# lmchion/PowerGridworld

Measured on AMD Instinct MI355X. Metric: agent-env-steps/sec at batch 65536, 5-agent scenario, 1/2/4/8 MI355X, higher is better.
Workload: dtype f64; 1 GPU; C4: 5-agent coordinated buildings (building+PV+storage) + IEEE-13 power flow + voltage-violation reward; pf_convergence=opendss, batch_per_gpu=65536, global_batch=65536, episode_steps=286, parallelism=env-sharded x1 (no collective on the step path)

## Files before the change

powergridworld_amd/csrc/pgw_pf.hip:

```cpp
#include <algorithm>
#include <cstdlib>
#include <cmath>
#include <type_traits>
#include <atomic>
#include <vector>

#include "pgw_common.h"

static std::atomic<bool> g_pf_trace_on{false};

namespace pgw {

template <int B, int E, class F>
__device__ __forceinline__ void static_for(F&& f) {
  if constexpr (B < E) {
    f(std::integral_constant<int, B>{});
    static_for<B + 1, E>(f);
  }
}

template <int M> struct PFBlock {
  static constexpr int kTri = M * (M + 1) / 2;
  static constexpr int kU0re = 3 * kTri, kU0im = kU0re + M, kU0sum = kU0im + M;
  static constexpr int kLo2 = kU0sum + M, kMn2 = kLo2 + M, kMx2 = kMn2 + M;
// ... 1740 lines not shown
    }
#pragma unroll
    for (int q = 0; q < kRq; ++q) {
      const int x = x0 + lane + 64 * q;
      if (x < z.n_rows * S) sh.rows[(x / S) * kWaveRowStride + (x - (x / S) * S)] = v[q];
    }
  }
  __builtin_amdgcn_fence(__ATOMIC_RELEASE, "wavefront");
  __builtin_amdgcn_wave_barrier();
  __builtin_amdgcn_fence(__ATOMIC_ACQUIRE, "wavefront");
}

__device__ __forceinline__ void od_wave_rows(const ODWaveShared& sh, int M, int r0, int r1, double pjr,
                                             double pji, double cjr, double cji, double& err, double& amin) {
  int lane = threadIdx.x & 63;
  asm volatile("" : "+v"(lane));
  const bool newer = lane >= 32;
  const int r = min(r0 + (lane & 31), max(r1 - 1, 0));
  const bool on = r0 + (lane & 31) < r1;
  const double* R = sh.rows + r * kWaveRowStride;
  double vr = R[0], vi = R[1];
#pragma unroll
  for (int k = 0; k < PGW_PF_MAX_M; ++k) {
    if (k >= M) break;
    const double gr = R[2 + k], gi = R[2 + M + k];
    const double pr = wave_bcast(pjr, k), pi = wave_bcast(pji, k);
    const double cr = wave_bcast(cjr, k), ci = wave_bcast(cji, k);
    const double jx = newer ? cr : pr, jy = newer ? ci : pi;
    vr = fma(gr, jx, vr);
    vi = fma(gr, jy, vi);
    vr = fma(-gi, jy, vr);
    vi = fma(gi, jx, vi);
  }
  const double mg = od_mag(fma(vi, vi, vr * vr));
  const double mn = wave_xor(mg, 32);
  const bool prev_lane = on && !newer;
  err = od_max(err, prev_lane ? fabs(mn - mg) : 0.0);
  amin = fmin(amin, prev_lane ? mg : __builtin_huge_val());
}

__device__ int od_wave_solve(const ODWaveArgs& z_, const ODWaveShared& sh_, double pc, double qc, double& v0r,
                             double& v0i) {
  int lane = threadIdx.x & 63;
  asm volatile("" : "+v"(lane));
  const ODWaveArgs& z = z_;
  const ODWaveShared& sh = sh_;
  const int M = z.m, T = M * (M + 1) / 2;
  const int i = min(lane, M - 1);
  const double sr0 = sh.el[0][i], si0 = sh.el[1][i], fr = sh.el[2][i], fi = sh.el[3][i];
  const double y0r = sh.el[4][i], y0i = sh.el[5][i], esc = sh.el[6][i];
  const bool node = lane < M && ((z.node_mask >> i) & 1);
  const double s_r = fma(fr, pc, sr0), s_i = fma(fi, qc, si0);
  const double* st = sh.st;
  const double u0re = sh.el[7][i], u0sum = sh.el[8][i];
  double ur = fma(qc, st[2 * (2 * M + i)], fma(pc, st[2 * (M + i)], st[2 * i]));
  double ui = fma(qc, st[2 * (2 * M + i) + 1], fma(pc, st[2 * (M + i) + 1], st[2 * i + 1]));
  const int c1 = 3 * M + i;
  double pjr = fma(qc, st[2 * (2 * M + c1)], fma(pc, st[2 * (M + c1)], st[2 * c1]));
  double pji = fma(qc, st[2 * (2 * M + c1) + 1], fma(pc, st[2 * (M + c1) + 1], st[2 * c1 + 1]));
  const double tol_lo = z.tol * (1.0 + 0x1p-30);
  const bool bounded = z.n_rep < z.n_rows;
  int it = 1, my_it = 1;
  bool conv_ok = false, done = z.max_iter <= 1;
  while (!done) {
    ++it;
    const double m2 = fma(ui, ui, ur * ur);
    double mc = fmin(fmax(m2, z.mn2), z.mx2);
    mc = (m2 <= z.lo2) ? 1.0 : mc;
    const double g = fast_rcp(mc);
    const double cr = fma(s_r, g, -y0r), ci = fma(s_i, g, -y0i);
    const double cjr = fma(cr, ur, -(ci * ui)), cji = fma(cr, ui, ci * ur);
    const double cjs = cjr + cji;
    double A = u0re, Bs = 0.0, C = u0sum;
    int ie = i;
    asm volatile("" : "+v"(ie));
    const double* wk = &sh.w[0][0][0] + ie;
#pragma unroll
    for (int k = 0; k < PGW_PF_MAX_M; ++k) {
      if (k < M) {
        A = fma(wk[k * PGW_PF_MAX_M], wave_bcast(cjr, k), A);
        Bs = fma(wk[(PGW_PF_MAX_M + k) * PGW_PF_MAX_M], wave_bcast(cji, k), Bs);
        C = fma(wk[(2 * PGW_PF_MAX_M + k) * PGW_PF_MAX_M], wave_bcast(cjs, k), C);
      }
    }
    const double nr = A - Bs, ni = (C - A) - Bs;
    bool hit = false;
    double err = 0.0, amin = __builtin_huge_val();
    {
      const double e2 = esc * esc;
      const double a2 = fma(ni, ni, nr * nr) * e2, b2 = fma(ui, ui, ur * ur) * e2;
      hit = node && fabs(a2 - b2) > tol_lo * fma(0.5, a2 + b2, 1.0);
    }
    const bool need = it >= z.min_iter && __ballot(hit) == 0ull;
    if (need) {
      const double mo = od_mag(fma(ui, ui, ur * ur)) * esc;
      const double mn = od_mag(fma(ni, ni, nr * nr)) * esc;
      err = node ? fabs(mn - mo) : 0.0;
      amin = node ? mo : __builtin_huge_val();
    }
    ur = nr;
    ui = ni;
    int d = 0;
    if (need) {
      double dsum = 0.0, jsum = 0.0;
#pragma unroll
      for (int k = 0; k < PGW_PF_MAX_M; ++k) {
        if (k >= M) break;
        const double cx = wave_bcast(cjr, k), cy = wave_bcast(cji, k);
        const double px = wave_bcast(pjr, k), py = wave_bcast(pji, k);
        dsum += fabs(cx - px) + fabs(cy - py);
        jsum += fabs(px) + fabs(py);
      }
      dsum = wave_uni(fma(0x1p-40, jsum + dsum, dsum));
      jsum = wave_uni(fma(0x1p-40, jsum, jsum));
      for (int r0 = 0; r0 < z.n_rep; r0 += 32)
        od_wave_rows(sh, M, r0, min(r0 + 32, z.n_rep), pjr, pji, cjr, cji, err, amin);
      double lo = wave_uni(wave_max(err)), am = wave_uni(wave_min(amin));
      d = __builtin_amdgcn_readfirstlane(od_decide(z, !bounded, it, lo, am, dsum, jsum));
      if (d < 0) {
        for (int r0 = z.n_rep; r0 < z.n_rows; r0 += 32)
          od_wave_rows(sh, M, r0, min(r0 + 32, z.n_rows), pjr, pji, cjr, cji, err, amin);
        lo = wave_uni(wave_max(err));
        am = wave_uni(wave_min(amin));
        d = __builtin_amdgcn_readfirstlane(od_decide(z, true, it, lo, am, dsum, jsum));
      }
    }
    pjr = cjr;
    pji = cji;
    my_it = it;
    conv_ok = d > 0;
    done = d > 0 || it >= z.max_iter;
  }
  const double* B = z.block + 3 * T + 6 * M;
  double vr = B[2 * M], vi = B[2 * M + 1];
#pragma unroll 4
  for (int k = 0; k < M; ++k) {
    const double gr = B[k], gi = B[M + k];
    const double jr = wave_bcast(pjr, k), ji = wave_bcast(pji, k);
    vr = fma(gr, jr, vr);
    vi = fma(gr, ji, vi);
    vr = fma(-gi, ji, vr);
    vi = fma(gi, jr, vi);
  }
  v0r = vr;
  v0i = vi;
  return conv_ok ? my_it : -my_it;
}

struct StepOdArgs {
  pgw_coord_params p;
  ODWaveArgs z;
};
template <bool WT, bool INL>
__global__ void __launch_bounds__(64 * PGW_MAX_AGENTS) __attribute__((amdgpu_waves_per_eu(7))) k_coord_step_od(StepOdArgs A_, pgw_coord_step_info s,
                                                                       int64_t n, pgw_coord_buffers b, double pv_ob,
                                                                       StdDerived dv, CoordPFArgs c, ODVLook o) {
  auto put = [](auto* q, auto v) {
    if constexpr (WT) st_wt(q, v);
    else *q = v;
  };
  const StepOdArgs& A = PGW_KERNARG0(StepOdArgs);
  const pgw_coord_params& p = A.p;
  const ODWaveArgs& z = A.z;
  const int a = threadIdx.x >> 6, lane = threadIdx.x & 63;
  const int64_t e = (int64_t)blockIdx.x * 64 + lane;
  const bool valid = e < n;
  __shared__ double s_pow[PGW_MAX_AGENTS][64];
  __shared__ double s_share[64];
  __shared__ int s_served[64];
  if (blockIdx.x == 0 && threadIdx.x == 0) b.od_count[(b.od_parity & 1) ^ 1] = 0;
  const ODVLook ol = {o.resp_v, o.resp_x0, o.resp_inv_h, o.resp_nseg, 0};
  double rw = 0.0;
  StdAgentInEarly in[1];
  double* xp = b.x + (int64_t)a * 5 * n + e;
  double* socp = b.soc + (int64_t)a * n + e;
  if (valid) {
    const double* ap = b.action.ptr + a * b.act_stride_agent + e * b.action.s_env;
#pragma unroll
    for (int j = 0; j < 8; ++j) in[0].av[j] = ld_act(ap + j * b.action.s_dim);
    in[0].soc = *socp;
#pragma unroll
    for (int z = 0; z < 5; ++z) in[0].xs[z] = xp[z * n];
    std_agent_compute<1, 1>(p, dv, s, pv_ob, in, [&](int, const double (&v)[1]) {
      s_pow[a][lane] = v[0];
      put(b.agent_power + (int64_t)a * n + e, v[0]);
    });
  }
  __syncthreads();
  double pc = 0.0;
  ODVRec rec;
  bool cell = false;
  if (valid) {
    double* op = b.obs.ptr + a * b.obs_stride_agent + e * b.obs.s_env;
    std_agent_compute<1, 2>(p, dv, s, pv_ob, in, [&](int slot, const double (&v)[1]) {
      if (slot < kSlotSoc) {
        put(xp + slot * n, v[0]);
        if (slot == kSlotX + 4 && a == 0) {
#pragma unroll
          for (int ag = 0; ag < PGW_MAX_AGENTS; ++ag) {
            const int cs = ag < c.n_agents ? c.agent_ctrl[ag] : -1;
            const double pa = ag < c.n_agents ? s_pow[ag][lane] * 1.0 : 0.0;
            pc = (cs == 0) ? pc + pa : pc;
          }
          int r = 0;
          cell = !o.timing_only && od_resp_v_cell(ol, pc, 0.0, r);
          if (cell) rec = od_resp_v_load(ol, r);
        }
      } else if (slot == kSlotSoc) put(socp, v[0]);
      else if (slot < kSlotPower) {
        if constexpr (WT) st_wt(op + (slot - kSlotObs) * b.obs.s_dim, v[0]);
        else st_obs(op + (slot - kSlotObs) * b.obs.s_dim, v[0]);
      } else {
        rw = v[0];
      }
    });
  }
  if (a == 0) {
    double2 vf = make_double2(0.0, 0.0);
    int it = 0;
    bool served = valid && cell && od_resp_v_chain(ol, pc, rec, vf, it);
    if constexpr (INL) {
      __shared__ ODWaveShared s_solve;
      uint64_t left = __ballot(valid && !served && !o.timing_only);
      if (left) {
        if (lane == 0) atomicAdd(b.od_count + (b.od_parity & 1), __popcll(left));
        od_wave_stage(z, s_solve);
        __shared__ double s_rw[64];
        s_rw[lane] = rw;
        do {
          const int L = __builtin_ctzll(left);
          left &= left - 1;
          double v0r, v0i;
          const int its = od_wave_solve(z, s_solve, wave_bcast(pc, L), 0.0, v0r, v0i);
          if (lane == L) {
            vf = make_double2(v0r, v0i);
            it = its;
            served = true;
          }
        } while (left);
        rw = s_rw[lane];
      }
    }
    double share = 0.0;
    if (served) {
      const double v0 = sqrt(fma(vf.y, vf.y, vf.x * vf.x));
      if (b.v_out) put(b.v_out + e, v0);
      if (b.iters) put(b.iters + e, (int32_t)it);
      if (c.coordinated) {
        const double vv = pymax(pymax(0.0, c.vv_lo - v0), v0 - c.vv_hi);
        if (b.vv) put(b.vv + e, vv);
        share = (vv * c.vv_penalty) / (double)c.n_agents;
      }
    }
    const bool need = !INL && valid && !served && !o.timing_only;
    const uint64_t m = __ballot(need);
    if (m) {
      const int first = __builtin_ctzll(m);
      int base = 0;
      if (lane == first) base = atomicAdd(b.od_count + (b.od_parity & 1), __popcll(m));
      base = __shfl(base, first);
      if (need) b.od_list[base + __popcll(m & ((1ull << lane) - 1ull))] = (int32_t)e;
    }
    s_share[lane] = share;
    s_served[lane] = served ? 1 : 0;
  }
  __syncthreads();
  if (!valid) return;
  const bool fin = c.coordinated && s_served[lane];
  put(b.reward + (int64_t)a * n + e, fin ? rw + (-s_share[lane]) : rw);
}

template <int M, bool LOOP>
__global__ void __launch_bounds__(kBlock) k_coord_pf_od_list(CoordPFArgs c, PFArgs a, ODArgs o, pgw_pf_tables t,
                                                             int64_t n, pgw_coord_buffers b) {
  const int32_t cnt = b.od_count[b.od_parity & 1];
  if ((int64_t)blockIdx.x * kBlock >= cnt) return;
  __shared__ ODShared<M> sh;
  if constexpr (LOOP) {
    for (int64_t base = (int64_t)blockIdx.x * kBlock; base < cnt; base += (int64_t)gridDim.x * kBlock) {
      const int64_t i = base + threadIdx.x;
      const bool valid = i < cnt;
      const int64_t e = valid ? (int64_t)b.od_list[i] : 0;
      coord_pf_od_env<M, pgw_coord_buffers, false, true>(c, a, o, t, n, b, e, valid, sh);
      __syncthreads();
    }
  } else {
    const int64_t i = (int64_t)blockIdx.x * kBlock + threadIdx.x;
    const bool valid = i < cnt;
    const int64_t e = valid ? (int64_t)b.od_list[i] : 0;
    coord_pf_od_env<M, pgw_coord_buffers, false, true>(c, a, o, t, n, b, e, valid, sh);
  }
}

template <int M, class IO = double>
__global__ void __launch_bounds__(kBlock) k_pf_solve_od(PFArgs a, ODArgs o, pgw_pf_tables t, int64_t n,
                                                        const IO* __restrict__ ctrl_p,
                                                        const IO* __restrict__ ctrl_q,
                                                        IO* __restrict__ v_out,
                                                        int32_t* __restrict__ iters) {
  const int64_t e = (int64_t)blockIdx.x * kBlock + threadIdx.x;
  const bool valid = e < n;
  __shared__ ODShared<M> sh;
  ODStage<M> stg;
  const bool table = o.resp != nullptr && t.U_out == nullptr;
  const bool rows_lds = od_rows_lds<M>(a.n_out);
  const bool qfast = table && v_out == nullptr && o.resp_q && rows_lds && o.resp_rows != 0 &&
                     (od_q_slot(o, 0) >= 0 || o.resp_v_row == 0);
  double rv[kOdRowQ];
  PFSolver<M, true, false> S;
  if (!qfast) {
    if (!table) od_stage_load<M>(o, o.start, stg);
    if (rows_lds) od_rows_issue<M>(t, a.n_out, rv);
    S.load(a, t.block);
  }
  double cp[PGW_PF_MAX_CTRL], cq[PGW_PF_MAX_CTRL];
#pragma unroll
  for (int c = 0; c < PGW_PF_MAX_CTRL; ++c) {
    cp[c] = (valid && c < a.n_ctrl && ctrl_p) ? (double)ctrl_p[(int64_t)c * n + e] : 0.0;
    cq[c] = (valid && c < a.n_ctrl && ctrl_q) ? (double)ctrl_q[(int64_t)c * n + e] : 0.0;
  }
  S.powers(a, cp, cq, 1.0);
  double ir[M], ii[M], v0r, v0i;
#pragma unroll
  for (int k = 0; k < M; ++k) ir[k] = ii[k] = 0.0;
  int it = 0;
  double2 vf = make_double2(0.0, 0.0);
  int rec = 0;
  double tq = 0.0;
  uint64_t qm = ~0ull;
  bool served, blk_fast = false;
  if (qfast) {
    served = valid && od_q_find(o, S.pc, S.qc, it, rec, tq, qm);
    if (served && o.resp_v) {
      const double2* vr = reinterpret_cast<const double2*>(o.resp_v) + (int64_t)rec * (PGW_OD_VREC / 2);
      vf = od_rec_j(vr[3], vr[4], vr[5], tq);
    }
    blk_fast = !__syncthreads_or(valid && !served);
    if (!blk_fast) {
      od_rows_issue<M>(t, a.n_out, rv);
      S.load(a, t.block);
      if (served) od_resp_at<M>(o, rec, tq, ir, ii, vf);
    } else {
#pragma unroll
      for (int q = 0; q < kOdRowQ; ++q) rv[q] = 0.0;
    }
  } else {
    served = valid && table && od_resp_lookup<M>(o, S.pc, S.qc, ir, ii, it, vf, rec, tq);
    if (served && o.resp_q) qm = od_q_cand(o.resp_q[(int64_t)rec * o.resp_q_stride + 5]);
  }
  const bool need = valid && !served;
  od_fallback<M>(S, o, o.start, stg, table, sh, need, ir, ii, it);
  v0r = v0i = 0.0;
  if (!blk_fast) pf_node0<M>(v0r, v0i, S.w, ir, ii);
  if (served && o.resp_v_row == 0) {
    v0r = vf.x;
    v0i = vf.y;
  }
  double m2_0 = fma(v0i, v0i, v0r * v0r);
  if (o.resp_q) {
    const int q0 = od_q_slot(o, 0);
    if (served && q0 >= 0) m2_0 = od_q_m2(o, rec, q0, tq);
  }
  const double v0 = sqrt(m2_0);
  const double vf2 = fma(vf.y, vf.y, vf.x * vf.x);
  if (valid && t.U_out) {
#pragma unroll
    for (int k = 0; k < M; ++k) {
      t.U_out[2 * (e * M + k)] = S.ur[k];
      t.U_out[2 * (e * M + k) + 1] = S.ui[k];
    }
  }
  double vmn = v0, vmx = v0;
  const double* srow = (rows_lds && !blk_fast) ? od_rows_put<M>(sh, a.n_out, rv) : nullptr;
  if (v_out || !rows_lds) {
    const double vfm = sqrt(vf2);
    pf_rows_out<M>(t, rows_lds, srow, a.n_out, ir, ii, [&](int ro, double v) {
      v = (served && ro == o.resp_v_row) ? vfm : v;
      const int qs = od_q_slot(o, ro);
      if (served && qs >= 0) v = sqrt(od_q_m2(o, rec, qs, tq));
      if (valid && v_out) v_out[(int64_t)ro * n + e] = (IO)v;
      vmn = (v < vmn) ? v : vmn;
      vmx = (v > vmx) ? v : vmx;
    });
  } else {
    double mn2 = m2_0, mx2 = mn2;
    auto ext = [&](int ro, double m2) {
      m2 = (served && ro == o.resp_v_row) ? vf2 : m2;
      const int qs = od_q_slot(o, ro);
      if (served && qs >= 0) {
        if (!((qm >> qs) & 1ull)) return;
        m2 = od_q_m2(o, rec, qs, tq);
      }
      mn2 = (m2 < mn2) ? m2 : mn2;
      mx2 = (m2 > mx2) ? m2 : mx2;
    };
    const uint64_t cand = o.resp_rows | (o.resp_v_row > 0 ? 1ull << o.resp_v_row : 0ull);
    if (blk_fast) {
      uint64_t m = a.n_out < 64 ? cand & ((1ull << a.n_out) - 1ull) & ~1ull : cand & ~1ull;
      while (m) {
        const int ro = __builtin_ctzll(m);
        m &= m - 1;
        ext(ro, 0.0);
      }
    } else if (rows_lds && o.resp_rows != 0 && __ballot(valid && !served) == 0ull) {
      pf_rows_mask2<M>(srow, a.n_out, cand, ir, ii, ext);
    } else {
      pf_rows_out<M, false>(t, rows_lds, srow, a.n_out, ir, ii, ext);
    }
    vmn = sqrt(mn2);
    vmx = sqrt(mx2);
  }
  if (!valid) return;
  if (a.n_out > 0) {
    if (v_out) v_out[e] = (IO)v0;
    if (t.v_min_out) t.v_min_out[e] = vmn;
    if (t.v_max_out) t.v_max_out[e] = vmx;
  }
  if (iters) iters[e] = it;
}

template <int M>
__global__ void __launch_bounds__(kBlock) k_pf_od_probe(const PFArgs* __restrict__ args_h, ODArgs o,
// ... 232 lines not shown
  const double x = v[e];
  const double l = x - lo, u = hi - x;
  const double viol = ((l < 0.0) ? l : 0.0) + ((u < 0.0) ? u : 0.0);
  const double y = scale * viol;
  out[e] = -(y * y);
}

static int32_t check_od(const pgw_pf_params& p, const pgw_pf_tables& t, const char* who) {
  const pgw_pf_od* d = t.od;
  PGW_REQUIRE(p.m == 14 && uniform_band(p) && p.n_ctrl <= 1 && !t.load_scale && !t.U_init,
              "%s: the OpenDSS fast path needs m = 14, one voltage band, <= 1 controllable slot and no "
              "load_scale / U_init (use pgw_pf_solve_general)", who);
  PGW_REQUIRE(d->n_rows >= 0 && d->n_rows <= PGW_PF_OD_MAX_ROWS && d->n_rep >= 0 && d->n_rep <= d->n_rows,
              "%s: od n_rep %d / n_rows %d (<= %d)", who, d->n_rep, d->n_rows, PGW_PF_OD_MAX_ROWS);
  PGW_REQUIRE(d->start && (d->n_rows == 0 || (d->rows_V0 && d->rows_G)), "%s: od start / rows missing", who);
  PGW_REQUIRE(d->min_iter >= 2 && p.max_iter >= 1 && d->tol >= 0.0, "%s: od min_iter / max_iter / tol", who);
  return PGW_OK;
}

#define PGW_PF_DISPATCH(p, t, fn, ...)                                     \
  do {                                                                     \
    const bool ub_ = uniform_band(p), gc_ = (p).n_ctrl > 1 || (t).load_scale; \
    switch ((p).m) {                                                       \
      case 8: return fn<8, false, true, true>(__VA_ARGS__);                \
      case 14:                                                             \
        if (ub_ && !gc_ && (p).n_out <= 1)                                 \
          return fn<14, true, false, false>(__VA_ARGS__);                  \
        if (ub_ && !gc_) return fn<14, true, false, true>(__VA_ARGS__);    \
        return fn<14, false, true, true>(__VA_ARGS__);                     \
      default: return fn<16, false, true, true>(__VA_ARGS__);              \
    }                                                                      \
  } while (0)

}

using namespace pgw;

constexpr int kOdListGrid = 1 << 30;
static int initial_od_list_grid() {
  const char* v = getenv("PGW_OD_LIST_GRID");
  const int g = v ? atoi(v) : 0;
  return g > 0 ? g : kOdListGrid;
}
static const int g_od_list_grid = initial_od_list_grid();
static bool initial_step_wt() {
  const char* v = getenv("PGW_STEP_WT");
  return v && v[0] == '1';
}
static const bool g_step_wt = initial_step_wt();
static const bool g_step_nolookup = getenv("PGW_STEP_NOLOOKUP") && getenv("PGW_STEP_NOLOOKUP")[0] == '1';
static const bool g_step_nop = getenv("PGW_STEP_NOP") && getenv("PGW_STEP_NOP")[0] == '1';
static const bool g_step_list = getenv("PGW_STEP_LIST") && getenv("PGW_STEP_LIST")[0] == '1';
static const bool g_step_nolist = getenv("PGW_STEP_NOLIST") && getenv("PGW_STEP_NOLIST")[0] == '1';
static ODWaveArgs make_wave_args(const PFArgs& a, const ODArgs& o, const pgw_pf_params& pf,
                                 const pgw_pf_tables& t) {
  ODWaveArgs z = {};
  for (int k = 0; k < PGW_PF_MAX_M; ++k) {
    z.sr0[k] = a.sr0[k];
    z.si0[k] = a.si0[k];
    z.fr[k] = a.fr[k];
    z.fi[k] = a.fi[k];
    z.y0r[k] = o.y0r[k];
    z.y0i[k] = o.y0i[k];
    z.esc[k] = o.esc[k];
  }
  z.lo2 = a.lo2;
  z.mn2 = a.mn2;
  z.mx2 = a.mx2;
  z.tol = o.tol;
  z.gamma = o.gamma;
  z.eps = o.eps;
  z.gmax = o.gmax;
  z.gsrc = o.gsrc;
  z.block = t.block;
  z.start = o.start;
  z.rows_V0 = o.rows_V0;
  z.rows_G = o.rows_G;
  z.m = pf.m;
  z.min_iter = o.min_iter;
  z.n_rep = o.n_rep;
  z.n_rows = o.n_rows;
  z.max_iter = o.max_iter;
  z.node_mask = o.node_mask;
  return z;
}
__global__ void k_step_nop(int* p) {
  if (p && threadIdx.x == 1000) *p = 0;
}

static int32_t launch_coord_agents(const pgw_coord_params& p, const pgw_coord_step_info& s, int64_t n,
                                   const pgw_coord_buffers& b, double pv_ob, bool std_layout, hipStream_t st) {
  if (std_layout)
    launch_timed(PGW_T_COORD_AGENTS, k_coord_agents_std<pgw_coord_buffers>, dim3(grid_for(n), p.n_agents),
                 dim3(kBlock), st, p, s, n, b, pv_ob, make_std_derived(p));
  else
    launch_timed(PGW_T_COORD_AGENTS, k_coord_agents, dim3(grid_for(n), p.n_agents), dim3(kBlock), st, p, s, n,
                 b);
  return check_launch("k_coord_agents");
}

template <class Bufs>
static int32_t coord_step(const pgw_coord_params* p, const pgw_pf_params* pf, const pgw_pf_tables* pft,
                          const pgw_coord_step_info* s, int64_t n, const Bufs& b, void* stream) {
  constexpr bool kF32 = std::is_same<Bufs, pgw_coord_buffers_f32>::value;
  PGW_REQUIRE(p && pf && pft && s && n >= 0, "pgw_coord_step: null argument");
  PGW_REQUIRE(p->n_agents >= 1 && p->n_agents <= PGW_MAX_AGENTS, "pgw_coord_step: bad n_agents");
  PGW_REQUIRE(p->n_comp >= 1 && p->n_comp <= 3, "pgw_coord_step: bad n_comp");
  PGW_REQUIRE(b.action.ptr && b.obs.ptr && b.reward && b.agent_power,
              "pgw_coord_step: null buffer");
  PGW_REQUIRE(pft->block, "pgw_coord_step: null PF block");
  PGW_REQUIRE(!pft->load_scale && !pft->U_init, "pgw_coord_step: load_scale / U_init not supported");
  PGW_REQUIRE(pf->m >= 1 && pf->m <= PGW_PF_MAX_M && pf->m == padded_m(pf->m),
              "pgw_coord_step: pf m=%d not padded", pf->m);
  PGW_REQUIRE(pf->n_out >= 1 && p->vv_row >= 0 && p->vv_row < pf->n_out,
              "pgw_coord_step: bad vv_row");
  PGW_REQUIRE(pft->G && pft->V0, "pgw_coord_step: missing G/V0");
  PGW_REQUIRE(pf->max_iter >= 1, "pgw_coord_step: max_iter < 1");
  PGW_REQUIRE(pf->n_ctrl >= 0 && pf->n_ctrl <= PGW_PF_MAX_CTRL, "pgw_coord_step: bad n_ctrl");
  for (int a = 0; a < p->n_agents; ++a)
    PGW_REQUIRE(p->agent_ctrl[a] < pf->n_ctrl, "pgw_coord_step: agent_ctrl out of range");
  for (int c = 0; c < p->n_comp; ++c) {
    int k = p->comp_order[c];
    PGW_REQUIRE(k >= 0 && k <= 2, "pgw_coord_step: bad comp_order");
    if (k == 0) PGW_REQUIRE(b.x && p->act_bld >= 0 && p->bld.n_obs <= PGW_BLD_MAX_OBS, "pgw_coord_step: building");
    if (k == 2) PGW_REQUIRE(b.soc && p->act_bat >= 0, "pgw_coord_step: storage");
  }
  if (n == 0) return PGW_OK;
  hipStream_t st = (hipStream_t)stream;
  const bool std_layout = coord_is_std(*p);
  PGW_REQUIRE(std_layout || !kF32,
              "pgw_coord_step_f32: needs the standard C4 agent layout (building/pv/storage at 0/6/7)");
  if (pft->od) {
    const int32_t rc_od = check_od(*pf, *pft, "pgw_coord_step");
    if (rc_od) return rc_od;
  }
  const double pv_ob = p->pv.rescale ? (2.0 * std::min(std::max(-s->pv_pmax, p->pv.obs_low), p->pv.obs_high)
                                        - (p->pv.obs_low + p->pv.obs_high)) / (p->pv.obs_high - p->pv.obs_low)
                                     : -s->pv_pmax;
  CoordPFArgs c = {};
  c.n_agents = p->n_agents;
  c.coordinated = p->coordinated;
  c.vv_row = p->vv_row;
  for (int a = 0; a < p->n_agents; ++a) c.agent_ctrl[a] = p->agent_ctrl[a];
  c.vv_lo = p->vv_lo;
  c.vv_hi = p->vv_hi;
  c.vv_penalty = p->vv_penalty;
  const PFArgs a = make_pf_args(*pf, *pft);
  if constexpr (!kF32) {
    if (pft->od && b.od_list && b.od_count && !g_pf_trace_on.load()) {
      const ODArgs o = make_od_args(*pft->od, pf->max_iter);
      if (std_layout && o.resp_v && o.resp_v_row == 0 && pf->n_out == 1 && p->vv_row == 0) {
        const ODVLook lk = {o.resp_v, o.resp_x0, o.resp_inv_h, o.resp_nseg, g_step_nolookup ? 1 : 0};
        const StepOdArgs sa = {*p, make_wave_args(a, o, *pf, *pft)};
        const dim3 grid((unsigned)((n + 63) / 64)), block(64 * p->n_agents);
        if (!g_step_list) {
          if (g_step_wt)
            launch_timed(PGW_T_COORD_AGENTS, k_coord_step_od<true, true>, grid, block, st, sa, *s, n, b, pv_ob,
                         make_std_derived(*p), c, lk);
          else
            launch_timed(PGW_T_COORD_AGENTS, k_coord_step_od<false, true>, grid, block, st, sa, *s, n, b, pv_ob,
                         make_std_derived(*p), c, lk);
          return check_launch("k_coord_step_od");
        }
        if (g_step_wt)
          launch_timed(PGW_T_COORD_AGENTS, k_coord_step_od<true, false>, grid, block, st, sa, *s, n, b, pv_ob,
                       make_std_derived(*p), c, lk);
        else
          launch_timed(PGW_T_COORD_AGENTS, k_coord_step_od<false, false>, grid, block, st, sa, *s, n, b, pv_ob,
                       make_std_derived(*p), c, lk);
        int32_t rc = check_launch("k_coord_step_od");
        if (rc) return rc;
        if (g_step_nop) hipLaunchKernelGGL(k_step_nop, dim3(1), dim3(64), 0, st, (int*)nullptr);
        if (g_step_nolist) return PGW_OK;
        if (g_od_list_grid >= grid_for(n))
          launch_timed(PGW_T_COORD_PF, k_coord_pf_od_list<14, false>, dim3((unsigned)grid_for(n)),
                       dim3(kBlock), st, c, a, o, *pft, n, b);
        else
          launch_timed(PGW_T_COORD_PF, k_coord_pf_od_list<14, true>, dim3((unsigned)g_od_list_grid),
                       dim3(kBlock), st, c, a, o, *pft, n, b);
        return check_launch("k_coord_pf_od_list");
      }
    }
    if (b.od_count) {
      const hipError_t me = hipMemsetAsync(b.od_count + ((b.od_parity & 1) ^ 1), 0, sizeof(int32_t), st);
      PGW_REQUIRE(me == hipSuccess, "pgw_coord_step: od_count reset: %s", hipGetErrorString(me));
    }
  }
  bool done = false;
  if constexpr (kF32) {
    if (std_layout && pairs_ok(b, n)) {
      launch_timed(PGW_T_COORD_AGENTS, k_coord_agents_std_x2<Bufs>, dim3(grid_for(n / 2), p->n_agents),
                   dim3(kBlock), st, *p, *s, n, b, pv_ob, make_std_derived(*p));
      done = true;
    }
  }
  if (done) {
  } else if (std_layout) {
    launch_timed(PGW_T_COORD_AGENTS, k_coord_agents_std<Bufs>, dim3(grid_for(n), p->n_agents),
                 dim3(kBlock), st, *p, *s, n, b, pv_ob, make_std_derived(*p));
  } else if constexpr (!kF32) {
    launch_timed(PGW_T_COORD_AGENTS, k_coord_agents, dim3(grid_for(n), p->n_agents), dim3(kBlock),
                 st, *p, *s, n, b);
  }
  int32_t rc = check_launch("k_coord_agents");
  if (rc) return rc;
  if (g_step_nop) hipLaunchKernelGGL(k_step_nop, dim3(1), dim3(64), 0, st, (int*)nullptr);
  hipStream_t pst = st;
  if (pft->od) {
    if (g_pf_trace_on.load())
      launch_timed(PGW_T_COORD_PF, k_coord_pf_od<14, Bufs, true>, dim3(grid_for(n)), dim3(kBlock), pst, c, a,
                   make_od_args(*pft->od, pf->max_iter), *pft, n, b);
    else
      launch_timed(PGW_T_COORD_PF, k_coord_pf_od<14, Bufs>, dim3(grid_for(n)), dim3(kBlock), pst, c, a,
                   make_od_args(*pft->od, pf->max_iter), *pft, n, b);
    return check_launch("k_coord_pf_od");
  }
  PGW_PF_DISPATCH(*pf, *pft, launch_coord_pf, c, a, *pft, n, b, pst);
}

static int32_t coord_step_general(const pgw_coord_params* p, const pgw_pfg_params* pf,
                                  const pgw_pfg_tables* pft, const pgw_coord_step_info* s, int64_t n,
                                  const pgw_coord_buffers& b, void* stream) {
  PGW_REQUIRE(p && pf && pft && s && n >= 0, "pgw_coord_step_general: null argument");
  PGW_REQUIRE(p->n_agents >= 1 && p->n_agents <= PGW_MAX_AGENTS, "pgw_coord_step_general: bad n_agents");
  PGW_REQUIRE(p->n_comp >= 1 && p->n_comp <= 3, "pgw_coord_step_general: bad n_comp");
  PGW_REQUIRE(b.action.ptr && b.obs.ptr && b.reward && b.agent_power, "pgw_coord_step_general: null buffer");
  PGW_REQUIRE(pf->n_out >= 1 && p->vv_row >= 0 && p->vv_row < pf->n_out, "pgw_coord_step_general: bad vv_row");
  for (int a = 0; a < p->n_agents; ++a)
    PGW_REQUIRE(p->agent_ctrl[a] < pf->n_ctrl, "pgw_coord_step_general: agent_ctrl out of range");
  for (int c = 0; c < p->n_comp; ++c) {
    int k = p->comp_order[c];
    PGW_REQUIRE(k >= 0 && k <= 2, "pgw_coord_step_general: bad comp_order");
    if (k == 0) PGW_REQUIRE(b.x && p->act_bld >= 0 && p->bld.n_obs <= PGW_BLD_MAX_OBS, "pgw_coord_step_general: building");
    if (k == 2) PGW_REQUIRE(b.soc && p->act_bat >= 0, "pgw_coord_step_general: storage");
  }
  if (n == 0) return PGW_OK;
  const double pv_ob = p->pv.rescale ? (2.0 * std::min(std::max(-s->pv_pmax, p->pv.obs_low), p->pv.obs_high)
                                        - (p->pv.obs_low + p->pv.obs_high)) / (p->pv.obs_high - p->pv.obs_low)
                                     : -s->pv_pmax;
  if (b.od_count) {
    const hipError_t me = hipMemsetAsync(b.od_count + ((b.od_parity & 1) ^ 1), 0, sizeof(int32_t),
                                         (hipStream_t)stream);
    PGW_REQUIRE(me == hipSuccess, "pgw_coord_step_general: od_count reset: %s", hipGetErrorString(me));
  }
  int32_t rc = launch_coord_agents(*p, *s, n, b, pv_ob, coord_is_std(*p), (hipStream_t)stream);
  if (rc) return rc;
  PFGCoord c = {};
  c.agent_power = b.agent_power;
  c.reward = b.reward;
  c.vv = b.vv;
  c.n_agents = p->n_agents;
  c.vv_row = p->vv_row;
  c.coordinated = p->coordinated;
  for (int a = 0; a < p->n_agents; ++a) c.agent_ctrl[a] = p->agent_ctrl[a];
  c.vv_lo = p->vv_lo;
  c.vv_hi = p->vv_hi;
  c.vv_penalty = p->vv_penalty;
  return solve_general(pf, pft, n, nullptr, nullptr, b.v_out, b.iters, c, stream);
}

extern "C" {

int32_t pgw_coord_step_general(const pgw_coord_params* p, const pgw_pfg_params* pf,
                               const pgw_pfg_tables* pft, const pgw_coord_step_info* s, int64_t n,
                               pgw_coord_buffers b, void* stream) {
  return coord_step_general(p, pf, pft, s, n, b, stream);
}

int32_t pgw_pf_padded_m(int32_t m) { return padded_m(m); }

int32_t pgw_voltage_band_penalty(int64_t n, const double* v, double lo, double hi, double scale,
                                 double* out, void* stream) {
  PGW_REQUIRE(v && out && n >= 0, "pgw_voltage_band_penalty: null argument");
  if (n == 0) return PGW_OK;
  hipLaunchKernelGGL(k_band_penalty, dim3(grid_for(n)), dim3(kBlock), 0, (hipStream_t)stream, n, v, lo,
                     hi, scale, out);
  return check_launch("k_band_penalty");
}

int64_t pgw_pf_od_probe_args_size(int32_t n_hours) {
  return n_hours <= 0 ? 0 : (int64_t)n_hours * (int64_t)sizeof(PFArgs);
}

int32_t pgw_pf_od_probe(const pgw_pf_params* p_hours, int32_t n_hours, const pgw_pf_tables* t,
                        const double* start_h, int32_t lanes_per_hour, int64_t n, const double* P,
                        double* J_out, uint64_t* sig_out, int32_t* it_out, void* args_buf, void* stream) {
  PGW_REQUIRE(p_hours && t && t->block && t->od && start_h && P && J_out && sig_out && it_out && args_buf,
              "pgw_pf_od_probe: null argument");
  PGW_REQUIRE(n_hours >= 1 && n >= 0 && lanes_per_hour > 0 && lanes_per_hour % kBlock == 0 &&
              n <= (int64_t)n_hours * lanes_per_hour,
              "pgw_pf_od_probe: n %lld lanes over %d hours of %d (a multiple of %d)", (long long)n, n_hours,
              lanes_per_hour, kBlock);
  std::vector<PFArgs> args(n_hours);
  for (int h = 0; h < n_hours; ++h) {
    const int32_t rc = check_od(p_hours[h], *t, "pgw_pf_od_probe");
    if (rc) return rc;
    PGW_REQUIRE(p_hours[h].m == p_hours[0].m && p_hours[h].n_ctrl == p_hours[0].n_ctrl &&
                p_hours[h].max_iter == p_hours[0].max_iter, "pgw_pf_od_probe: hours differ in shape");
    args[h] = make_pf_args(p_hours[h], *t);
  }
  if (n == 0) return PGW_OK;
  hipStream_t st = (hipStream_t)stream;
  PGW_REQUIRE(hipMemcpyAsync(args_buf, args.data(), sizeof(PFArgs) * n_hours, hipMemcpyHostToDevice, st) ==
                  hipSuccess && hipStreamSynchronize(st) == hipSuccess,
              "pgw_pf_od_probe: argument upload failed");
  hipLaunchKernelGGL(k_pf_od_probe<14>, dim3(grid_for(n)), dim3(kBlock), 0, st,
                     reinterpret_cast<const PFArgs*>(args_buf), make_od_args(*t->od, p_hours[0].max_iter), *t,
// ... 164 lines not shown
```

Measured before the change: 14.80 billion agent-env-steps/s.

## Move voltage lookup and inline power-flow solve into a dedicated extra wave

Adds one extra wavefront per block that handles the aggregate-power sum, voltage lookup, inline OpenDSS wave solve, violation penalty and od_list append, while the agent waves only do the building/PV/storage compute and the final reward write. Previously agent wave 0 did both its own agent work and the power-flow work, which serialized that wave relative to the others. Agent ctrl flags and lookup scalars are pinned to scalar registers. The trade-off is a larger block (n_agents+1 waves) and an extra barrier, which may lower occupancy and makes the agent waves wait at the barrier for the lookup wave.

```diff
diff --git a/powergridworld_amd/csrc/pgw_pf.hip b/powergridworld_amd/csrc/pgw_pf.hip
--- a/powergridworld_amd/csrc/pgw_pf.hip
+++ b/powergridworld_amd/csrc/pgw_pf.hip
@@ -1916,7 +1916,7 @@
   ODWaveArgs z;
 };
 template <bool WT, bool INL>
-__global__ void __launch_bounds__(64 * PGW_MAX_AGENTS) __attribute__((amdgpu_waves_per_eu(7))) k_coord_step_od(StepOdArgs A_, pgw_coord_step_info s,
+__global__ void __launch_bounds__(64 * (PGW_MAX_AGENTS + 1)) __attribute__((amdgpu_waves_per_eu(7))) k_coord_step_od(StepOdArgs A_, pgw_coord_step_info s,
                                                                        int64_t n, pgw_coord_buffers b, double pv_ob,
                                                                        StdDerived dv, CoordPFArgs c, ODVLook o) {
   auto put = [](auto* q, auto v) {
@@ -1927,111 +1927,118 @@
   const pgw_coord_params& p = A.p;
   const ODWaveArgs& z = A.z;
   const int a = threadIdx.x >> 6, lane = threadIdx.x & 63;
+  const bool look = __builtin_amdgcn_readfirstlane(a) == c.n_agents;
   const int64_t e = (int64_t)blockIdx.x * 64 + lane;
   const bool valid = e < n;
   __shared__ double s_pow[PGW_MAX_AGENTS][64];
   __shared__ double s_share[64];
   __shared__ int s_served[64];
-  if (blockIdx.x == 0 && threadIdx.x == 0) b.od_count[(b.od_parity & 1) ^ 1] = 0;
-  const ODVLook ol = {o.resp_v, o.resp_x0, o.resp_inv_h, o.resp_nseg, 0};
-  double rw = 0.0;
-  StdAgentInEarly in[1];
-  double* xp = b.x + (int64_t)a * 5 * n + e;
-  double* socp = b.soc + (int64_t)a * n + e;
-  if (valid) {
-    const double* ap = b.action.ptr + a * b.act_stride_agent + e * b.action.s_env;
-#pragma unroll
-    for (int j = 0; j < 8; ++j) in[0].av[j] = ld_act(ap + j * b.action.s_dim);
-    in[0].soc = *socp;
-#pragma unroll
-    for (int z = 0; z < 5; ++z) in[0].xs[z] = xp[z * n];
-    std_agent_compute<1, 1>(p, dv, s, pv_ob, in, [&](int, const double (&v)[1]) {
-      s_pow[a][lane] = v[0];
-      put(b.agent_power + (int64_t)a * n + e, v[0]);
-    });
-  }
+  if (!look) {
+    if (blockIdx.x == 0 && threadIdx.x == 0) b.od_count[(b.od_parity & 1) ^ 1] = 0;
+    double rw = 0.0;
+    StdAgentInEarly in[1];
+    double* xp = b.x + (int64_t)a * 5 * n + e;
+    double* socp = b.soc + (int64_t)a * n + e;
+    if (valid) {
+      const double* ap = b.action.ptr + a * b.act_stride_agent + e * b.action.s_env;
+#pragma unroll
+      for (int j = 0; j < 8; ++j) in[0].av[j] = ld_act(ap + j * b.action.s_dim);
+      in[0].soc = *socp;
+#pragma unroll
+      for (int z = 0; z < 5; ++z) in[0].xs[z] = xp[z * n];
+      std_agent_compute<1, 1>(p, dv, s, pv_ob, in, [&](int, const double (&v)[1]) {
+        s_pow[a][lane] = v[0];
+        put(b.agent_power + (int64_t)a * n + e, v[0]);
+      });
+    }
+    __syncthreads();
+    if (valid) {
+      double* op = b.obs.ptr + a * b.obs_stride_agent + e * b.obs.s_env;
+      std_agent_compute<1, 2>(p, dv, s, pv_ob, in, [&](int slot, const double (&v)[1]) {
+        if (slot < kSlotSoc) put(xp + slot * n, v[0]);
+        else if (slot == kSlotSoc) put(socp, v[0]);
+        else if (slot < kSlotPower) {
+          if constexpr (WT) st_wt(op + (slot - kSlotObs) * b.obs.s_dim, v[0]);
+          else st_obs(op + (slot - kSlotObs) * b.obs.s_dim, v[0]);
+        } else {
+          rw = v[0];
+        }
+      });
+    }
+    __syncthreads();
+    if (!valid) return;
+    const bool fin = c.coordinated && s_served[lane];
+    put(b.reward + (int64_t)a * n + e, fin ? rw + (-s_share[lane]) : rw);
+    return;
+  }
+  ODVLook ol = {o.resp_v, o.resp_x0, o.resp_inv_h, o.resp_nseg, 0};
+  int ctrl[PGW_MAX_AGENTS];
+#pragma unroll
+  for (int ag = 0; ag < PGW_MAX_AGENTS; ++ag) {
+    ctrl[ag] = c.agent_ctrl[ag];
+    asm volatile("" : "+s"(ctrl[ag]));
+  }
+  asm volatile("" : "+s"(ol.resp_x0), "+s"(ol.resp_inv_h), "+s"(ol.resp_nseg));
   __syncthreads();
   double pc = 0.0;
   ODVRec rec;
   bool cell = false;
   if (valid) {
-    double* op = b.obs.ptr + a * b.obs_stride_agent + e * b.obs.s_env;
-    std_agent_compute<1, 2>(p, dv, s, pv_ob, in, [&](int slot, const double (&v)[1]) {
-      if (slot < kSlotSoc) {
-        put(xp + slot * n, v[0]);
-        if (slot == kSlotX + 4 && a == 0) {
-#pragma unroll
-          for (int ag = 0; ag < PGW_MAX_AGENTS; ++ag) {
-            const int cs = ag < c.n_agents ? c.agent_ctrl[ag] : -1;
-            const double pa = ag < c.n_agents ? s_pow[ag][lane] * 1.0 : 0.0;
-            pc = (cs == 0) ? pc + pa : pc;
-          }
-          int r = 0;
-          cell = !o.timing_only && od_resp_v_cell(ol, pc, 0.0, r);
-          if (cell) rec = od_resp_v_load(ol, r);
+#pragma unroll
+    for (int ag = 0; ag < PGW_MAX_AGENTS; ++ag) {
+      const int cs = ag < c.n_agents ? ctrl[ag] : -1;
+      const double pa = ag < c.n_agents ? s_pow[ag][lane] * 1.0 : 0.0;
+      pc = (cs == 0) ? pc + pa : pc;
+    }
+    int r = 0;
+    cell = !o.timing_only && od_resp_v_cell(ol, pc, 0.0, r);
+    if (cell) rec = od_resp_v_load(ol, r);
+  }
+  double2 vf = make_double2(0.0, 0.0);
+  int it = 0;
+  bool served = valid && cell && od_resp_v_chain(ol, pc, rec, vf, it);
+  if constexpr (INL) {
+    __shared__ ODWaveShared s_solve;
+    uint64_t left = __ballot(valid && !served && !o.timing_only);
+    if (left) {
+      if (lane == 0) atomicAdd(b.od_count + (b.od_parity & 1), __popcll(left));
+      od_wave_stage(z, s_solve);
+      do {
+        const int L = __builtin_ctzll(left);
+        left &= left - 1;
+        double v0r, v0i;
+        const int its = od_wave_solve(z, s_solve, wave_bcast(pc, L), 0.0, v0r, v0i);
+        if (lane == L) {
+          vf = make_double2(v0r, v0i);
+          it = its;
+          served = true;
         }
-      } else if (slot == kSlotSoc) put(socp, v[0]);
-      else if (slot < kSlotPower) {
-        if constexpr (WT) st_wt(op + (slot - kSlotObs) * b.obs.s_dim, v[0]);
-        else st_obs(op + (slot - kSlotObs) * b.obs.s_dim, v[0]);
-      } else {
-        rw = v[0];
-      }
-    });
-  }
-  if (a == 0) {
-    double2 vf = make_double2(0.0, 0.0);
-    int it = 0;
-    bool served = valid && cell && od_resp_v_chain(ol, pc, rec, vf, it);
-    if constexpr (INL) {
-      __shared__ ODWaveShared s_solve;
-      uint64_t left = __ballot(valid && !served && !o.timing_only);
-      if (left) {
-        if (lane == 0) atomicAdd(b.od_count + (b.od_parity & 1), __popcll(left));
-        od_wave_stage(z, s_solve);
-        __shared__ double s_rw[64];
-        s_rw[lane] = rw;
-        do {
-          const int L = __builtin_ctzll(left);
-          left &= left - 1;
-          double v0r, v0i;
-          const int its = od_wave_solve(z, s_solve, wave_bcast(pc, L), 0.0, v0r, v0i);
-          if (lane == L) {
-            vf = make_double2(v0r, v0i);
-            it = its;
-            served = true;
-          }
-        } while (left);
-        rw = s_rw[lane];
-      }
-    }
-    double share = 0.0;
-    if (served) {
-      const double v0 = sqrt(fma(vf.y, vf.y, vf.x * vf.x));
-      if (b.v_out) put(b.v_out + e, v0);
-      if (b.iters) put(b.iters + e, (int32_t)it);
-      if (c.coordinated) {
-        const double vv = pymax(pymax(0.0, c.vv_lo - v0), v0 - c.vv_hi);
-        if (b.vv) put(b.vv + e, vv);
-        share = (vv * c.vv_penalty) / (double)c.n_agents;
-      }
-    }
-    const bool need = !INL && valid && !served && !o.timing_only;
-    const uint64_t m = __ballot(need);
-    if (m) {
-      const int first = __builtin_ctzll(m);
-      int base = 0;
-      if (lane == first) base = atomicAdd(b.od_count + (b.od_parity & 1), __popcll(m));
-      base = __shfl(base, first);
-      if (need) b.od_list[base + __popcll(m & ((1ull << lane) - 1ull))] = (int32_t)e;
-    }
-    s_share[lane] = share;
-    s_served[lane] = served ? 1 : 0;
-  }
+      } while (left);
+    }
+  }
+  double share = 0.0;
+  if (served) {
+    const double v0 = sqrt(fma(vf.y, vf.y, vf.x * vf.x));
+    if (b.v_out) put(b.v_out + e, v0);
+    if (b.iters) put(b.iters + e, (int32_t)it);
+    if (c.coordinated) {
+      const double vv = pymax(pymax(0.0, c.vv_lo - v0), v0 - c.vv_hi);
+      if (b.vv) put(b.vv + e, vv);
+      share = (vv * c.vv_penalty) / (double)c.n_agents;
+    }
+  }
+  const bool need = !INL && valid && !served && !o.timing_only;
+  const uint64_t m = __ballot(need);
+  if (m) {
+    const int first = __builtin_ctzll(m);
+    int base = 0;
+    if (lane == first) base = atomicAdd(b.od_count + (b.od_parity & 1), __popcll(m));
+    base = __shfl(base, first);
+    if (need) b.od_list[base + __popcll(m & ((1ull << lane) - 1ull))] = (int32_t)e;
+  }
+  s_share[lane] = share;
+  s_served[lane] = served ? 1 : 0;
   __syncthreads();
-  if (!valid) return;
-  const bool fin = c.coordinated && s_served[lane];
-  put(b.reward + (int64_t)a * n + e, fin ? rw + (-s_share[lane]) : rw);
 }
 
 template <int M, bool LOOP>
@@ -2570,7 +2577,8 @@
       if (std_layout && o.resp_v && o.resp_v_row == 0 && pf->n_out == 1 && p->vv_row == 0) {
         const ODVLook lk = {o.resp_v, o.resp_x0, o.resp_inv_h, o.resp_nseg, g_step_nolookup ? 1 : 0};
         const StepOdArgs sa = {*p, make_wave_args(a, o, *pf, *pft)};
-        const dim3 grid((unsigned)((n + 63) / 64)), block(64 * p->n_agents);
+        static_assert(64 * (PGW_MAX_AGENTS + 1) <= 1024, "k_coord_step_od: a block of PGW_MAX_AGENTS + 1 waves");
+        const dim3 grid((unsigned)((n + 63) / 64)), block(64 * (p->n_agents + 1));
         if (!g_step_list) {
           if (g_step_wt)
             launch_timed(PGW_T_COORD_AGENTS, k_coord_step_od<true, true>, grid, block, st, sa, *s, n, b, pv_ob,
```

Result: faster. 15.52 billion agent-env-steps/s (median of 6 runs) (+4.9%).
